# niessner/Opt

Measured on AMD Instinct MI355X. Metric: PCG iters/s, GN solve of image_warping 4096^2, higher is better.
Workload: dtype f32; 1 GPU; image_warping 4096x4096 float, gaussNewtonGPU, 400 PCG iterations per GN step (synthetic cat512-style constraints, border pinned); parallelism=single GPU, step=one Opt_ProblemStep (1 GN iteration)

## Files before the change

opt_amd/csrc/energy_image_warping.hip:

```cpp
#include "energy.h"
#include "iw_device.h"
#include "iw_step.h"
#include "iw_iter.h"
#include "pcg_ring.h"
#include "iw_onchip.h"
#include <cstdint>

namespace optamd {
namespace {

template <class T>
struct ImageWarpingOps : EnergyOps<T> {
    IWArgs<T> A{};
    int cus = 256;
    bool useLattice = true;
    int forceRows = 0, maxWorkgroups = 1 << 30, maxExchangePeriod = 1 << 20;
    ImageWarpingOps(const unsigned* dims) {
        A.W = (int)dims[0]; A.H = (int)dims[1];
        this->usePreconditioner = true;
        this->addUnknown(0, (long)A.W * A.H, 2); this->addUnknown(1, (long)A.W * A.H, 1);
        HIP_CHECK(hipMalloc((void**)&A.flags, (size_t)A.W * A.H));
        HIP_CHECK(hipMalloc((void**)&A.cs, (size_t)A.W * A.H * 2 * sizeof(T)));
        int dev = 0; HIP_CHECK(hipGetDevice(&dev));
        HIP_CHECK(hipDeviceGetAttribute(&cus, hipDeviceAttributeMultiprocessorCount, dev));
        if (const char* e = getenv("OPT_AMD_LATTICE")) useLattice = atoi(e) != 0;
        if (const char* e = getenv("OPT_AMD_SLAB_PERIOD")) maxExchangePeriod = std::max(1, atoi(e));
        if (const char* e = getenv("OPT_AMD_ITER_ROWS")) forceRows = std::max(0, atoi(e));
        if (const char* e = getenv("OPT_AMD_ITER_MAXWG")) maxWorkgroups = std::max(1, atoi(e));
        if (const char* e = getenv("OPT_AMD_ONCHIP_FLAT")) ocFlatMax = std::max(0, atoi(e));
        HIP_CHECK(hipMalloc((void**)&dNotLattice, sizeof(int)));
        HIP_CHECK(hipHostMalloc((void**)&hNotLattice, 64)); *hNotLattice = 0;
        HIP_CHECK(hipEventCreateWithFlags(&bindEvent, hipEventDisableTiming));
    }
    ~ImageWarpingOps() override {
        (void)hipHostFree(hNotLattice); (void)hipEventDestroy(bindEvent);
        (void)hipFree(A.flags); (void)hipFree(A.cs); (void)hipFree(dNotLattice);
// ... 172 lines not shown
        const int gx = divUp(A.W, kStrip);
        int gy, rowsPerGroup;
        splitRows(A.yEnd - A.yBegin, gx, cus * occReset, gy, rowsPerGroup);
        FuseArgs<T> F{};
        F.resetB = b; F.resetPre = pre; F.resetR = r; F.resetZ = z; F.resetBNum = bNum.partials; F.resetQ = q.partials;
        ScopedKernel k(ctx, "PCGStep1+PCGStep2_2ndHalf");
        iw_applyJTJ<T, true, false, true><<<gx * gy, kBlock, 0, ctx.stream>>>(A, delta, nullptr, CtC, nullptr, rowsPerGroup, gx, gy, F);
        bNum.n = gx * gy; q.n = gx * gy;
        return true;
    }
    bool applyJTJFused(const T* pOld, const T* z, T* pNew, T* out, const T* CtC, Reduction* dot, const Reduction& bNum, const double* aNumOld,
                       double* aNumNext, LaunchCtx& ctx) override {
        FuseArgs<T> F{z, pNew, bNum.partials, bNum.n, aNumOld, aNumNext};
        launchApply(pOld, out, CtC, dot, ctx, &F);
        return true;
    }

    static const void* iterKernel(bool lat, bool lmLoop, bool flip, int mode) {
#define IWK(LAT, PRE, LMV, MODE) (flip ? (const void*)iw_pcgIter2<T, LAT, PRE, true, LMV, MODE> : (const void*)iw_pcgIter2<T, LAT, PRE, false, LMV, MODE>)
        if (lmLoop) return lat ? (mode == 1 ? IWK(true, 3, true, 1) : mode == 2 ? IWK(true, 3, true, 2) : IWK(true, 3, true, 0)) : IWK(false, 1, true, 0);
        if (lat) return mode == 1 ? IWK(true, 3, false, 1) : mode == 2 ? IWK(true, 3, false, 2) : IWK(true, 3, false, 0);
        return mode == 1 ? IWK(false, 2, false, 1) : mode == 2 ? IWK(false, 2, false, 2) : IWK(false, 2, false, 0);
#undef IWK
    }
    static int iterBlock(bool lat, bool lmLoop) { return sizeof(T) == 8 ? 256 : lat ? 768 : lmLoop ? 512 : 768; }
    int occIter[4] = {0, 0, 0, 0};
    PcgRing<T> ring; double* lmQState = nullptr;
    struct IterLoop {
        bool gn = false, lmRing = false;
        int sinceExchange = 0;
        int lmPrN = 0;
    } loop;
    bool iterAccepts(bool lmLoop) const { return fits32() && (!this->slab.active || (this->slab.ghost >= 2 && !lmLoop)); }
    IterTraits iterTraits(bool lmLoop) const override {
        IterTraits t;
        const bool ok = iterAccepts(lmLoop);
        t.stateExchange = ok;
        t.takesMail = ok && !lmLoop;
        t.postsItself = ok && !lmLoop && this->slab.active;
        t.slabAvailable = ok;
        return t;
    }
    void beginLoop(LaunchCtx& ctx) {
        resolveLattice();
        if (initPending) { if (initHint && !lattice) launchJtf(false, ctx); initHint = lattice; initPending = false; }
    }
    bool pcgIteration(const PcgIterArgs<T>& a, LaunchCtx& ctx) override {
        const bool lmLoop = a.CtC != nullptr;
        if (!a.pre || !iterAccepts(lmLoop)) return false;
        if (a.first) { beginLoop(ctx); loop = IterLoop{}; }
        PcgIterResult<T>& res = *a.result;
        int ext = 0;
        if (this->slab.active) {
            const int period = std::max(1, std::min(this->slab.ghost - 1, maxExchangePeriod)), j = loop.sinceExchange + 1;
            const bool due = j >= period;
            ext = due ? 0 : this->slab.ghost - j;
            loop.sinceExchange = due ? 0 : j;
            res.exchangeDue = due;
        }
        IWArgs<T> Ax = A;
        Ax.yBegin = std::max(0, A.yBegin - ext); Ax.yEnd = std::min(A.H, A.yEnd + ext);
        const int blk = iterBlock(lattice, lmLoop), L = (lmLoop ? 2 : 0) + (lattice ? 1 : 0);
        if (occIter[L] == 0) {
            HIP_CHECK(hipOccupancyMaxActiveBlocksPerMultiprocessor(&occIter[L], iterKernel(lattice, lmLoop, false, 0), blk, 0));
            occIter[L] = std::max(1, std::min(occIter[L], 8));
        }
        const int gx = divUp(A.W, (blk / kWave) * kSpan2);
        int gy, rowsPerGroup;
        splitRows(Ax.yEnd - Ax.yBegin, gx, cus * occIter[L], gy, rowsPerGroup);
        const bool gn = !lmLoop, lmRing = lmLoop && lattice;
        loop.gn = gn; loop.lmRing = lmRing;
        typename PcgRing<T>::Launch R{};
        if (gn || lmRing) {
            ring.allocate((size_t)A.W * A.H * 3, ctx.stream);
            R = ring.next(a.first != 0, a.afterReset != 0, a.rOld, a.pOld);
        } else { R.flip = ring.nextSweep(a.first != 0); R.pOld = a.pOld; R.rOld = a.rOld; R.pNew = a.pNew; }
        if (gn) {
            res.exchange[0] = R.pNew; res.nExchange = 1;
            if (R.k >= 1) { res.exchange[1] = const_cast<T*>(R.pOld); res.nExchange = 2; }
        }
        if (lmRing) {
            res.p = R.pNew; res.wroteDelta = R.deltaMode == 1;
            if (R.owedP) { res.owedP = R.owedP; res.owedAlpha = R.alphaOut; }
            if (!lmQState) {
                HIP_CHECK(hipMalloc((void**)&lmQState, sizeof(double) * (1 + 2 * (size_t)kMaxPartials)));
                HIP_CHECK(hipMemsetAsync(lmQState, 0, sizeof(double) * (1 + 2 * (size_t)kMaxPartials), ctx.stream));
            }
        }
        IterK<T> K{};
        K.rOld = R.rOld; K.pOld = R.pOld; K.rNew = a.rNew; K.pNew = R.pNew; K.delta = a.delta; K.deltaOut = a.deltaOut ? a.deltaOut : a.delta;
        K.pre = a.pre; K.first = a.first; K.deltaMode = R.deltaMode; K.alphaIn = R.alphaIn; K.alphaOut = R.alphaOut; K.rfree = R.rfree;
        K.CtC = a.CtC; K.b = a.b; K.q = a.q ? a.q->partials : nullptr; K.qTag = a.qTag; K.afterReset = a.afterReset;
        K.betaNum = a.betaNum.partials; K.nBetaNum = a.betaNum.n; K.betaDen = a.betaDen.partials; K.nBetaDen = a.betaDen.n;
        if (lmRing) {
            K.qState = lmQState; K.qInit = a.qInit;
            K.pr = lmQState + 1 + (size_t)(R.k & 1) * kMaxPartials; K.prPrev = lmQState + 1 + (size_t)((R.k & 1) ^ 1) * kMaxPartials; K.nPr = loop.lmPrN;
        }
        K.lmRadius = a.lmRadius; K.lmMin = a.lmMinDiag; K.lmMax = a.lmMaxDiag;
        K.aNumPrev = a.aNumPrev.partials; K.aDenPrev = a.aDenPrev.partials; K.s2Prev = a.s2Prev.partials; K.s3Prev = a.s3Prev.partials;
        K.nNum = a.aNumPrev.n; K.nDen = a.aDenPrev.n; K.n2 = a.s2Prev.n; K.n3 = a.s3Prev.n;
        K.aNum = a.aNum->partials; K.aDen = a.aDen->partials; K.s2 = a.s2->partials; K.s3 = a.s3->partials;
        K.ownBegin = A.yBegin; K.ownEnd = A.yEnd;
        K.mail = MailRefDev{a.mail.words, a.mail.world, a.mail.stride, a.mail.tag, a.mail.timeoutTicks, a.mail.errFlag};
        for (int t = 0; t < 16; ++t) K.post.dst[t] = a.post.dst[t];
        K.post.world = a.post.world; K.post.tag = a.post.tag; K.post.ticket = a.post.ticket;
        K.deltaZero = 0;
        if (deltaZero && !a.first && R.deltaMode != 2 && gn) { K.deltaZero = 1; deltaZero = false; }
        {
            ScopedKernel k(ctx, "PCGIteration");
            int rpg = rowsPerGroup, gxa = gx, gya = gy;
            void* kargs[] = {(void*)&Ax, (void*)&K, (void*)&rpg, (void*)&gxa, (void*)&gya};
            const int mode = ((gn || lmRing) && R.rfree == 1 && !a.first && !a.afterReset && !K.deltaZero) ? (R.deltaMode == 2 ? 1 : 2) : 0;
            HIP_CHECK(hipLaunchKernel(iterKernel(lattice, lmLoop, R.flip != 0, mode), dim3(gx * gy), dim3(blk), kargs, 0, ctx.stream));
        }
        a.aNum->n = a.aDen->n = a.s2->n = a.s3->n = gx * gy;
        if (a.q) a.q->n = lmRing ? 1 : gx * gy;
        loop.lmPrN = gx * gy;
        return true;
    }
    void addOwedTerm(T* delta, const T* p, const T* alpha, LaunchCtx& ctx) override {
        ScopedKernel k(ctx, "PCGStep2_delta");
        const long n = 3L * A.W * A.H;
        axpyDeferred<T><<<flatGrid(n), kBlock, 0, ctx.stream>>>(delta, p, alpha, n);
    }
    const T* pcgFinish(T* delta, LaunchCtx& ctx) override {
        if (deltaZero) { HIP_CHECK(hipMemsetAsync(delta, 0, ((size_t)A.W * A.H * 3 + 3) / 4 * 4 * sizeof(T), ctx.stream)); deltaZero = false; }
        if (!loop.gn) return nullptr;
        const long n = 3L * A.W * A.H;
        return ring.finish(delta, n, flatGrid(n), ctx);
    }
    bool finishUpdate(const T* delta, const Reduction& aNum, const Reduction& aDen, LaunchCtx& ctx) override {
        if (this->slab.active || !loop.gn) return false;
        ScopedKernel k(ctx, "PCGLinearUpdate");
        const long N = (long)A.W * A.H;
        iw_finishUpdate<T><<<flatGrid(N), kBlock, 0, ctx.stream>>>(const_cast<T*>(A.Offset), const_cast<T*>(A.Angle), deltaZero ? nullptr : delta, ring.pLast(), ring.termOwed() ? ring.pPrev() : nullptr,
                                                                   ring.alphaSlot(ring.iterIndex - 1), N, aNum.partials, aNum.n, aDen.partials, aDen.n);
        ring.settled(); deltaZero = false;
        return true;
    }
    bool supportsSlab() const override { return true; }
    long rowScalars(int img) const override { return (long)A.W * (img == 0 ? 2 : 1); }

    struct OcVariant { int rows; bool apLds, deltaGlb; const void* fn; size_t lds; int occ; };
    std::vector<OcVariant> ocVariants, ocVariantsLM, ocVariantsGeneral, ocVariantsGeneralLM;
    OnchipGuard guard;
    OnchipGuard* onChipGuard() override { return &guard; }
    int ocFlatMax = 256; long long* ocProf = nullptr;
    OnchipSync ocS{};
    void ocInit() {
        if (!ocVariants.empty()) return;
// ... 122 lines not shown
    void onChipApply(const T* delta, const double* verdict, bool , LaunchCtx& ctx) override {
        ScopedKernel k(ctx, "PCGLinearUpdate");
        const long N = (long)A.W * A.H;
        iw_applyDelta<T><<<flatGrid(N), kBlock, 0, ctx.stream>>>(const_cast<T*>(A.Offset), const_cast<T*>(A.Angle), delta, N, guard.bad, verdict, guard.hostErr, guard.stepWord());
        guard.launched = true;
    }
    std::string describe(int L, bool lmv, const OnChipLm<T>*) override {
        const Slab& sl = this->slab;
        const int rowsOwned = (sl.active ? sl.yEnd - sl.yBegin : A.H);
        char buf[1400];
        if (sl.active) { A.yBegin = sl.yBegin; A.yEnd = sl.yEnd; } else { A.yBegin = 0; A.yEnd = A.H; }
        int tX = 0, tY = 0;
        const bool eligible = guard.usable() && L > 0 && !(lmv && sl.active);
        const OcVariant* V = eligible ? ocSelect(tX, tY, lmv) : nullptr;
        int uX = 0, uY = 0; const OcVariant* U = nullptr;
        if (eligible && !V && maxWorkgroups < (1 << 30)) { const int keep = maxWorkgroups; maxWorkgroups = 1 << 30; U = ocSelect(uX, uY, lmv); maxWorkgroups = keep; }
        const bool ghostOk = !sl.active || sl.ghost >= 2;
        const long rowBytes = (long)A.W * 3 * (long)sizeof(T);
        const std::string cap = maxWorkgroups < (1 << 30) ? std::to_string(maxWorkgroups) + " (OPT_AMD_ITER_MAXWG: ranks share a GPU)" : std::string("none");
        if (V && ghostOk)
            snprintf(buf, sizeof buf, "path=on-chip (if UrShape is the unit lattice%s); onchip_rows_per_lane=%d; tiles=%dx%d of %d CUs; lds_bytes=%zu; slab_rows=%d; ghost_rows=%d; workgroup_cap=%s; "
                     "per_iteration_cross_rank=%s; fallback=one launch per PCG iteration (iw_pcgIter2)",
                     sl.active ? " and every rank and the communicator agree" : "", V->rows, tX, tY, cus, V->lds, rowsOwned, sl.active ? sl.ghost : 0, cap.c_str(),
                     sl.active ? "edge rows of A p as tagged words (2 x W x 3 scalars x 8 B per neighbour) + one rank hop of 4 doubles, inside the persistent launch" : "none");
        else {
            const std::string why = guard.whyOff() ? guard.whyOff() : (lmv && sl.active) ? "the LM variants are single-GPU" : !ghostOk ? "needs >= 2 ghost rows" :
                                    U ? "the workgroup cap -- without it: on-chip, " + std::to_string(U->rows) + " rows per lane, " + std::to_string(uX) + "x" + std::to_string(uY) + " tiles" :
                                    "the tiles do not fit one per CU (or the slab is no whole number of tiles)";
            const std::string cross = sl.active ? "one all-reduce of 4 doubles, and every " + std::to_string(std::max(1, sl.ghost - 1)) + " iterations " + std::to_string(2L * sl.ghost * rowBytes) +
                                                  " B of edge rows (the two newest search directions) per neighbour" : std::string("none");
            snprintf(buf, sizeof buf, "path=one launch per PCG iteration (iw_pcgIter2%s); why_not_on_chip=%s; slab_rows=%d; ghost_rows=%d; workgroup_cap=%s; per_iteration_cross_rank=%s",
                     lmv ? ", LM" : "", why.c_str(), rowsOwned, sl.active ? sl.ghost : 0, cap.c_str(), cross.c_str());
        }
        if (this->onChipLevel < 4) return buf;
        std::string d = buf;
        int gX = 0, gY = 0;
        const OcVariant* GV = (eligible && !sl.active) ? ocSelect(gX, gY, lmv, true) : nullptr;
        if (GV && lmv && gX * gY > ocFlatMax) GV = nullptr;
        if (GV) {
            if (V && ghostOk) d.replace(0, d.find(';'), "path=on-chip (unit-lattice UrShape: iw_onchipPcg, any other UrShape: iw_onchipPcgGeneral)");
            d += "; general_urshape=on-chip (iw_onchipPcgGeneral" + std::string(lmv ? ", LM" : "") + "), " + std::to_string(GV->rows) + " rows per lane, " + std::to_string(gX) + "x" + std::to_string(gY) +
                 " tiles, " + std::to_string(GV->lds) + " B of LDS";
        } else {
            const std::string why = guard.whyOff() ? guard.whyOff() : sl.active ? "row slabs take the on-chip solve on a unit lattice only" : L <= 0 ? "no PCG iterations" :
                                    "no general-UrShape variant fits one tile per CU (at most " + std::to_string(sizeof(T) == 4 ? 2048 : 1024) + " pixels per CU" + (lmv ? ", LM: at most " + std::to_string(ocFlatMax) + " tiles" : "") + ")";
            d += "; general_urshape=one launch per PCG iteration (iw_pcgIter2" + std::string(lmv ? ", LM" : "") + "); why_not_on_chip_general=" + why;
        }
        return d;
    }
    bool supportsDeferredSteps() const override { return !this->slab.active; }
    bool deltaMovable() const override { return !this->slab.active; }
};

template <class T> EnergyOps<T>* makeIW(const unsigned* dims) { return new ImageWarpingOps<T>(dims); }

}

EnergyInfo imageWarpingInfo() {
    EnergyInfo e;
    e.name = "image_warping"; e.nDims = 2; e.usePreconditioner = true; e.floatOnly = false; e.residualsPerElement = 10;
    e.params = {{ParamDecl::kUnknown, "Offset", "opt_float2", 0}, {ParamDecl::kUnknown, "Angle", "opt_float", 1},
                {ParamDecl::kArray, "UrShape", "opt_float2", 2},  {ParamDecl::kArray, "Constraints", "opt_float2", 3},
                {ParamDecl::kArray, "Mask", "opt_float", 4},      {ParamDecl::kScalar, "w_fitSqrt", "float", 5},
                {ParamDecl::kScalar, "w_regSqrt", "float", 6}};
    e.makeFloat = makeIW<float>; e.makeDouble = makeIW<double>;
    return e;
}

// ... 2 lines not shown
```

opt_amd/csrc/iw_device.h:

```cpp
#pragma once
#include "common.h"
#include <cstdint>

namespace optamd {
namespace {

template <class T> struct V2 { T x, y; };

constexpr uint8_t kActive = 1, kFit = 2;
constexpr int kCountShift = 2;

template <class T>
struct Q {
    T ox, oy, a;
    T c, s;
    T ux, uy;
    T on;
    T fw;
};
template <int DX, int DY, bool LATTICE, class T>
__device__ __forceinline__ void iw_pairQ(const Q<T>& c, const Q<T>& n, T& ax, T& ay, T& aa) {
    T Dcx, Dcy, Dnx, Dny;
    if (LATTICE) {
        Dcx = DX ? T(DX) * c.s : T(DY) * c.c;   Dcy = DX ? T(-DX) * c.c : T(DY) * c.s;
// ... 30 lines not shown
    const T jnx = -dx - Dnx * n.a, jny = -dy - Dny * n.a;
    PairOut<T> o;
    o.dx = jcx - jnx; o.dy = jcy - jny;
    o.tn = Dnx * jnx + Dny * jny;
    ax += n.on * o.dx; ay += n.on * o.dy;
    aa -= n.on * (Dcx * jcx + Dcy * jcy);
    return o;
}
template <class T>
__device__ __forceinline__ void iw_pairInherited(const PairOut<T>& o, T nOn, T& ax, T& ay, T& aa) {
    ax -= nOn * o.dx; ay -= nOn * o.dy;
    aa -= nOn * o.tn;
}
template <class T>
struct IWArgs {
    int W, H;
    int yBegin, yEnd;
    int gy0, Hg;
    const T* Offset; const T* Angle; const T* UrShape; const T* Constraints; const T* Mask;
    T w_fit, w_reg;
    uint8_t* flags;
    T* cs;
};


__device__ __forceinline__ float regCopy(float v) { float r; asm("v_mov_b32 %0, %1" : "=v"(r) : "v"(v)); return r; }
__device__ __forceinline__ int regCopy(int v) { int r; asm("v_mov_b32 %0, %1" : "=v"(r) : "v"(v)); return r; }
__device__ __forceinline__ double regCopy(double v) { return __hiloint2double(regCopy(__double2hiint(v)), regCopy(__double2loint(v))); }


typedef unsigned int iw_u2 __attribute__((ext_vector_type(2)));
typedef unsigned int iw_u4 __attribute__((ext_vector_type(4)));
__device__ __forceinline__ __amdgpu_buffer_rsrc_t iw_rsrc(const void* base) { return __builtin_amdgcn_make_buffer_rsrc(const_cast<void*>(base), 0, -1 , 0x00020000); }
__device__ __forceinline__ V2<float> bufLd2(__amdgpu_buffer_rsrc_t r, unsigned v, unsigned so, const float*) { const iw_u2 w = __builtin_amdgcn_raw_buffer_load_b64(r, (int)v, (int)so, 0); return V2<float>{__uint_as_float(w.x), __uint_as_float(w.y)}; }
__device__ __forceinline__ V2<double> bufLd2(__amdgpu_buffer_rsrc_t r, unsigned v, unsigned so, const double*) { const iw_u4 w = __builtin_amdgcn_raw_buffer_load_b128(r, (int)v, (int)so, 0); V2<double> o; __builtin_memcpy(&o, &w, 16); return o; }
__device__ __forceinline__ float bufLd1(__amdgpu_buffer_rsrc_t r, unsigned v, unsigned so, const float*) { return __uint_as_float(__builtin_amdgcn_raw_buffer_load_b32(r, (int)v, (int)so, 0)); }
__device__ __forceinline__ double bufLd1(__amdgpu_buffer_rsrc_t r, unsigned v, unsigned so, const double*) { const iw_u2 w = __builtin_amdgcn_raw_buffer_load_b64(r, (int)v, (int)so, 0); double o; __builtin_memcpy(&o, &w, 8); return o; }
__device__ __forceinline__ void bufSt2(__amdgpu_buffer_rsrc_t r, unsigned v, unsigned so, float x, float y) { __builtin_amdgcn_raw_buffer_store_b64(iw_u2{__float_as_uint(x), __float_as_uint(y)}, r, (int)v, (int)so, 0); }
__device__ __forceinline__ void bufSt2(__amdgpu_buffer_rsrc_t r, unsigned v, unsigned so, double x, double y) { const V2<double> o{x, y}; iw_u4 w; __builtin_memcpy(&w, &o, 16); __builtin_amdgcn_raw_buffer_store_b128(w, r, (int)v, (int)so, 0); }
__device__ __forceinline__ void bufSt1(__amdgpu_buffer_rsrc_t r, unsigned v, unsigned so, float x) { __builtin_amdgcn_raw_buffer_store_b32(__float_as_uint(x), r, (int)v, (int)so, 0); }
__device__ __forceinline__ void bufSt1(__amdgpu_buffer_rsrc_t r, unsigned v, unsigned so, double x) { iw_u2 w; __builtin_memcpy(&w, &x, 8); __builtin_amdgcn_raw_buffer_store_b64(w, r, (int)v, (int)so, 0); }
}
}
```

opt_amd/csrc/iw_iter.h:

```cpp
#pragma once
#include "iw_device.h"

namespace optamd {
namespace {

constexpr int kSpan2 = kWave - 4;
template <class T, bool LATTICE, int PRE, bool LM> struct IterBlk {
    static constexpr int value = sizeof(T) == 8 ? 256 : LATTICE ? 768 : (PRE == 2 && !LM) ? 768 : 512;
};

template <class T>
struct IterRaw {
    V2<T> ro, po, mo, u, co; T ra, pa, ma, ca, ang;
    int f, ok;
};
template <class T>
struct IterK {
    const T *rOld, *pOld; T *rNew, *pNew; T* delta; T* deltaOut;
    const T* pre;
    int first;
    int deltaMode; const T* alphaIn; T* alphaOut;
    int rfree;
    const T* CtC; const T* b; double* q; unsigned qTag; int afterReset; const double* betaNum; int nBetaNum; const double* betaDen; int nBetaDen;
    double* qState; double qInit;
    const double* prPrev; int nPr; double* pr;
    T lmRadius, lmMin, lmMax;
    const double *aNumPrev, *aDenPrev, *s2Prev, *s3Prev; int nNum, nDen, n2, n3;
    double *aNum, *aDen, *s2, *s3;
    int ownBegin, ownEnd;
    MailRefDev mail;
    MailPostDev post;
    int deltaZero;
};
template <class T>
struct IterBufs {
    __amdgpu_buffer_rsrc_t rOld, pOld, pNew, rNew, delta, deltaOut, angle, flags, pre, ctc, b, ur;
    unsigned x2, x1, x0;
    unsigned aPart;
};
template <class T, bool LATTICE, int PRE, bool LMV, bool FLIP>
__device__ __forceinline__ IterRaw<T> iw_iterLoad(const IWArgs<T>& A, const IterBufs<T>& B, bool xok, int y) {
    IterRaw<T> r;
    r.ok = xok && y >= 0 && y < A.H;
    const int yc = min(max(y, 0), A.H - 1);
    const unsigned row = (unsigned)(FLIP ? A.H - 1 - yc : yc) * (unsigned)A.W;
    const unsigned s2 = row * (unsigned)sizeof(V2<T>), s1 = row * (unsigned)sizeof(T), s1a = s1 + B.aPart;
    const T* tag = nullptr;
    r.f = __builtin_amdgcn_raw_buffer_load_b8(B.flags, (int)B.x0, (int)row, 0);
    r.ro = bufLd2(B.rOld, B.x2, s2, tag); r.ra = bufLd1(B.rOld, B.x1, s1a, tag);
    r.po = bufLd2(B.pOld, B.x2, s2, tag); r.pa = bufLd1(B.pOld, B.x1, s1a, tag);
    if (PRE == 1) { r.mo = bufLd2(B.pre, B.x2, s2, tag); r.ma = bufLd1(B.pre, B.x1, s1a, tag); }
    else { r.mo = V2<T>{0, 0}; r.ma = 0; }
    if (LMV) { r.co = bufLd2(B.ctc, B.x2, s2, tag); r.ca = bufLd1(B.ctc, B.x1, s1a, tag); } else { r.co = V2<T>{0, 0}; r.ca = 0; }
    r.ang = bufLd1(B.angle, B.x1, s1, tag);
    if (LATTICE) r.u = V2<T>{0, 0}; else r.u = bufLd2(B.ur, B.x2, s2, tag);
    return r;
}

template <bool RIGHT, bool LATTICE, class T> __device__ __forceinline__ void dppShiftConst(const Q<T>& p, Q<T>& q) {
    q.c = dppShift<RIGHT>(p.c); q.s = dppShift<RIGHT>(p.s); q.on = dppShift<RIGHT>(p.on);
    if (LATTICE) { q.ux = 0; q.uy = 0; } else { q.ux = dppShift<RIGHT>(p.ux); q.uy = dppShift<RIGHT>(p.uy); }
    q.fw = 0;
}
template <bool RIGHT, class T> __device__ __forceinline__ void dppShiftVec(const Q<T>& p, Q<T>& q) {
    q.ox = dppShift<RIGHT>(p.ox); q.oy = dppShift<RIGHT>(p.oy); q.a = dppShift<RIGHT>(p.a);
}
template <class T>
struct OldRow {
    Q<T> q;
    T rx, ry, ra, mx, my, ma;
    T cx, cy, ca;
    T p2x, p2y, p2a;
};
template <class T>
struct NewRow {
    Q<T> q;
    T rx, ry, ra, mx, my, ma;
    T cx, cy, ca;
    Q<T> lf, rt;
};

template <class T, bool LATTICE, int PRE, bool FLIP, bool LM = false, int MODE = 0>
__global__ __launch_bounds__((IterBlk<T, LATTICE, PRE, LM>::value), 1) void iw_pcgIter2(IWArgs<T> A, IterK<T> K, int rowsPerGroup, int gx, int gy) {
    static_assert(MODE == 0 || !LM || PRE == 3, "steady-state specialisations: the r-free loops (Gauss-Newton; Levenberg-Marquardt on a unit lattice)");
    static_assert(PRE >= 1 && PRE <= 3, "image_warping always preconditions (image_warping.t:10)");
    const int kDeltaMode = MODE == 1 ? 2 : MODE == 2 ? 1 : K.deltaMode, kRfree = MODE ? 1 : K.rfree;
    constexpr bool LMRF = LM && PRE == 3;
    constexpr int kBlk = IterBlk<T, LATTICE, PRE, LM>::value, kStripW = (kBlk / kWave) * kSpan2;
    __shared__ double scratch[5 * (kBlk / kWave + 1)];
    const long N = (long)A.W * A.H;
    const int bx = blockIdx.x % gx, by = blockIdx.x / gx;
    const int lane = threadIdx.x & (kWave - 1), wave = threadIdx.x >> 6;
    const int x = bx * kStripW + wave * kSpan2 + lane - 2;
    const bool xok = x >= 0 && x < A.W;
    const bool writer = xok && lane >= 2 && lane < 2 + kSpan2;
    const int lyBegin = FLIP ? A.H - A.yEnd : A.yBegin, lyEnd = FLIP ? A.H - A.yBegin : A.yEnd;
    const int yb = lyBegin + by * rowsPerGroup, ye = min(yb + rowsPerGroup, lyEnd);
    IterBufs<T> Bf;
    {
        const unsigned xc = (unsigned)min(max(x, 0), A.W - 1);
        Bf.x2 = xc * (unsigned)sizeof(V2<T>); Bf.x1 = xc * (unsigned)sizeof(T); Bf.x0 = xc; Bf.aPart = (unsigned)(2 * N * (long)sizeof(T));
        Bf.rOld = iw_rsrc(K.rOld); Bf.pOld = iw_rsrc(K.pOld); Bf.pNew = iw_rsrc(K.pNew); Bf.rNew = iw_rsrc(K.rNew); Bf.delta = iw_rsrc(K.delta); Bf.deltaOut = iw_rsrc(K.deltaOut);
        Bf.angle = iw_rsrc(A.Angle); Bf.flags = iw_rsrc(A.flags); Bf.pre = iw_rsrc(K.pre); Bf.ctc = iw_rsrc(K.CtC); Bf.b = iw_rsrc(K.b); Bf.ur = iw_rsrc(A.UrShape);
    }
    auto loadRow = [&](int y) { return iw_iterLoad<T, LATTICE, PRE, LM && PRE != 3, FLIP>(A, Bf, xok, y); };
    const IterRaw<T> raw0 = loadRow(yb - 2), raw1 = loadRow(yb - 1);
    IterRaw<T> rwA = loadRow(yb), rwB = loadRow(yb + 1), rwC = loadRow(yb + 2);
    T alpha = 0, beta = 0;
    const bool first = MODE ? false : K.first != 0;
    const bool restart = LM && MODE == 0 && K.afterReset != 0;
    if (restart) {
        const double* const ps[2] = {K.betaNum, K.betaDen}; const int ns[2] = {K.nBetaNum, K.nBetaDen}; double o2[2];
        sumPartialsN<2>(ps, ns, scratch, o2);
        const T bNum = (T)o2[0], bDen = (T)o2[1];
        beta = (bDen > T(0)) ? bNum / bDen : T(0);
    } else if (!first) {
        const double* const ps[4] = {K.aNumPrev, K.aDenPrev, K.s2Prev, K.s3Prev}; const int ns[4] = {K.nNum, K.nDen, K.n2, K.n3}; double o4[4]; double prD = 0;
        if (!LM && K.mail.words) {
            __shared__ double mailScr[4 + 1 + 64];
            pollMailSums<4>(K.mail, mailScr, o4);
        } else if constexpr (LMRF) {
            const double* const ps5[5] = {K.aNumPrev, K.aDenPrev, K.s2Prev, K.s3Prev, K.prPrev}; const int ns5[5] = {K.nNum, K.nDen, K.n2, K.n3, K.nPr}; double o5[5];
            sumPartialsN<5>(ps5, ns5, scratch, o5);
            o4[0] = o5[0]; o4[1] = o5[1]; o4[2] = o5[2]; o4[3] = o5[3]; prD = o5[4];
        } else sumPartialsN<4>(ps, ns, scratch, o4);
        const double aNumD = o4[0], aDenD = o4[1], s2 = o4[2], s3 = o4[3];
        const T aNum = (T)aNumD, aDen = (T)aDenD;
        alpha = (aDen > T(0)) ? aNum / aDen : T(0);
        if (LMRF && blockIdx.x == 0 && threadIdx.x == 0) {
            const double qNow = K.qState[0] + (double)alpha * (prD - 0.5 * (double)alpha * aDenD);
            K.qState[0] = qNow;
            if (K.qTag) storeTaggedPartial(K.q, 0, qNow, K.qTag); else K.q[0] = qNow;
        }
        const double bNumD = fmax(aNumD - 2.0 * (double)alpha * s2 + (double)alpha * (double)alpha * s3, 0.0);
        beta = (aNum > T(0)) ? (T)bNumD / aNum : T(0);
    }
    if (K.alphaOut && blockIdx.x == 0 && threadIdx.x == 0) { K.alphaOut[0] = alpha; K.alphaOut[2] = beta; }
    if (LMRF && (first || restart) && blockIdx.x == 0 && threadIdx.x == 0) K.qState[0] = first ? 0.0 : K.qInit;
    const T alpha2 = (kDeltaMode == 1) ? K.alphaIn[0] : T(0);
    const bool reconR = (!LM || LMRF) && kRfree == 1;
// ... 41 lines not shown
            if (reconR) { ix = iy = iTab[io]; ia = iTab[10 + cnt]; }
        } else if (PRE == 2) {
            o.mx = o.my = mTab[io]; o.ma = 0;
            if (!LM && reconR) { ix = iy = iTab[io]; ia = T(1); }
        } else {
            o.mx = w.mo.x; o.my = w.mo.y; o.ma = w.ma;
            if (!LM && reconR) { ix = T(1) / o.mx; iy = T(1) / o.my; ia = T(1) / o.ma; }
        }
        if ((!LM || LMRF) && LATTICE && kRfree) { o.p2x = w.ro.x; o.p2y = w.ro.y; o.p2a = w.ra; }
        if (reconR) {
            o.rx = (o.q.ox - betaOlder * w.ro.x) * ix; o.ry = (o.q.oy - betaOlder * w.ro.y) * iy; o.ra = (o.q.a - betaOlder * w.ra) * ia;
        }
    };
    auto applyA = [&](const Q<T>& c, const Q<T>& lf, const Q<T>& rt, const Q<T>& prev, const Q<T>& next, PairOut<T>& vert, T& ox, T& oy, T& oa, bool wantM, T& vertM, T& pa) {
        T ax = 0, ay = 0, aa = 0;
        T mh[2] = {0, 0}, mv[2] = {0, 0};
        const PairOut<T> hr = iw_pairFull<1, 0, LATTICE>(c, rt, ax, ay, aa, wantM ? mh : nullptr, A.w_reg);
        PairOut<T> hl; hl.dx = dppShift<true>(hr.dx); hl.dy = dppShift<true>(hr.dy); hl.tn = dppShift<true>(hr.tn);
        const T mhl = wantM ? dppShift<true>(mh[1]) : T(0);
        iw_pairInherited(hl, lf.on, ax, ay, aa);
        if (!FLIP) {
            const PairOut<T> vn = iw_pairFull<0, 1, LATTICE>(c, next, ax, ay, aa, wantM ? mv : nullptr, A.w_reg); iw_pairInherited(vert, prev.on, ax, ay, aa); vert = vn;
            if (wantM) { T t = rt.on * mh[0]; t += lf.on * mhl; t += next.on * mv[0]; t += prev.on * vertM; pa = t; vertM = mv[1]; }
        } else {
            iw_pairInherited(vert, prev.on, ax, ay, aa); vert = iw_pairFull<0, -1, LATTICE>(c, next, ax, ay, aa, wantM ? mv : nullptr, A.w_reg);
            if (wantM) { T t = rt.on * mh[0]; t += lf.on * mhl; t += prev.on * vertM; t += next.on * mv[0]; pa = t; vertM = mv[1]; }
        }
        ox = c.on * (w2 * ax + c.fw * c.ox); oy = c.on * (w2 * ay + c.fw * c.oy); oa = c.on * (w2 * aa);
    };
    PairOut<T> vOld{0, 0, 0}, vNew{0, 0, 0};
    T vOldM = 0, unusedM = 0;
    constexpr bool kDeltaEarly = MODE == 2 || (LM && !LMRF);
    struct DeltaPre { V2<T> o; T a; };
    auto loadDelta = [&](int y1) {
        DeltaPre d{V2<T>{0, 0}, 0};
        if constexpr (kDeltaEarly) {
            const int yc = min(max(y1, 0), A.H - 1);
            const unsigned rowE = (unsigned)(FLIP ? A.H - 1 - yc : yc) * (unsigned)A.W;
            const T* const tag = nullptr;
            d.o = bufLd2(Bf.delta, Bf.x2, rowE * (unsigned)sizeof(V2<T>), tag); d.a = bufLd1(Bf.delta, Bf.x1, rowE * (unsigned)sizeof(T) + Bf.aPart, tag);
            __builtin_amdgcn_sched_barrier(0);
        }
        return d;
    };
    auto trip = [&](int y, const OldRow<T>& oA, const OldRow<T>& oB, const OldRow<T>& oC,
                    const NewRow<T>& nA, const NewRow<T>& nB, NewRow<T>& nC, bool live, const DeltaPre& dPre) {
        nC.q = oB.q;
        nC.lf = Q<T>{}; nC.lf.on = dppShift<true>(oB.q.on);
        dppShiftConst<false, LATTICE>(oB.q, nC.rt);
        Q<T> lf = nC.lf, rt = nC.rt;
        dppShiftVec<false>(oB.q, rt);
        T ax, ay, aa, paB = 0;
        applyA(oB.q, lf, rt, oA.q, oC.q, vOld, ax, ay, aa, PRE == 2, vOldM, paB);
        if (LM) { ax += oB.cx * oB.q.ox; ay += oB.cy * oB.q.oy; aa += oB.ca * oB.q.a; }
        T maB = oB.ma, raB = oB.ra;
        if (PRE == 2) {
            const T sq = T(1) + sqrt(paB), ia = sq * sq;
            maB = T(1) / ia;
            if (!LM && reconR) raB = oB.ra * ia;
        }
        const T rx = keepR ? oB.rx : oB.rx - alpha * ax, ry = keepR ? oB.ry : oB.ry - alpha * ay, ra = keepR ? raB : raB - alpha * aa;
        nC.mx = oB.mx; nC.my = oB.my; nC.ma = maB;
        nC.cx = oB.cx; nC.cy = oB.cy; nC.ca = oB.ca;
        nC.rx = rx; nC.ry = ry; nC.ra = ra;
        const T zx = nC.mx * rx, zy = nC.my * ry, za = nC.ma * ra;
        nC.q.ox = zx + beta * oB.q.ox; nC.q.oy = zy + beta * oB.q.oy; nC.q.a = za + beta * oB.q.a;
        if (live && writer && y + 1 >= yb && y + 1 < ye) {
            const int yp = phys(y + 1);
            const unsigned rowE = (unsigned)yp * (unsigned)A.W, s2 = rowE * (unsigned)sizeof(V2<T>), s1a = rowE * (unsigned)sizeof(T) + Bf.aPart;
            const T* const tag = nullptr;
            const bool own = yp >= K.ownBegin && yp < K.ownEnd;
            if (own && !keepR && kDeltaMode != 2) {
                V2<T> d; T da;
// ... 9 lines not shown
                    }
                }
                d.x += alpha * oB.q.ox; d.y += alpha * oB.q.oy; da += alpha * oB.q.a;
                bufSt2(Bf.deltaOut, Bf.x2, s2, d.x, d.y); bufSt1(Bf.deltaOut, Bf.x1, s1a, da);
                if (LM && !LMRF) {
                    const V2<T> bo = bufLd2(Bf.b, Bf.x2, s2, tag); const T ba = bufLd1(Bf.b, Bf.x1, s1a, tag);
                    accQ += (double)(T(0.5) * (d.x * (rx + bo.x))) + (double)(T(0.5) * (d.y * (ry + bo.y))) + (double)(T(0.5) * (da * (ra + ba)));
                }
            }
            if (!kRfree) { bufSt2(Bf.rNew, Bf.x2, s2, rx, ry); bufSt1(Bf.rNew, Bf.x1, s1a, ra); }
            bufSt2(Bf.pNew, Bf.x2, s2, nC.q.ox, nC.q.oy); bufSt1(Bf.pNew, Bf.x1, s1a, nC.q.a);
        }
        Q<T> l2 = nB.lf, r2 = nB.rt;
        dppShiftVec<false>(nB.q, r2);
        T ox, oy, oa;
        applyA(nB.q, l2, r2, nA.q, nC.q, vNew, ox, oy, oa, false, unusedM, unusedM);
        if (LM) { ox += nB.cx * nB.q.ox; oy += nB.cy * nB.q.oy; oa += nB.ca * nB.q.a; }
        if (live && writer && y >= yb && phys(y) >= K.ownBegin && phys(y) < K.ownEnd) {
            accDen += (double)(nB.q.ox * ox + nB.q.oy * oy + nB.q.a * oa);
            if (LMRF) accQ += (double)nB.q.ox * (double)nB.rx + (double)nB.q.oy * (double)nB.ry + (double)nB.q.a * (double)nB.ra;
            const double mx = (double)nB.mx, my = (double)nB.my, ma = (double)nB.ma;
            const double rx2 = (double)nB.rx, ry2 = (double)nB.ry, ra2 = (double)nB.ra, ax2 = (double)ox, ay2 = (double)oy, az2 = (double)oa;
            const double mrx = mx * rx2, mry = my * ry2, mra = ma * ra2;
            accNum += mrx * rx2 + mry * ry2 + mra * ra2;
            acc2 += mrx * ax2 + mry * ay2 + mra * az2;
            acc3 += (mx * ax2) * ax2 + (my * ay2) * ay2 + (ma * az2) * az2;
        }
    };
    OldRow<T> o0, o1, o2;
    NewRow<T> n0{}, n1{}, n2{};
    makeOld(raw0, o0);
    makeOld(raw1, o1);
    { T t0 = 0, t1 = 0, t2 = 0, m0[2] = {0, 0}; vOld = iw_pairFull<0, FLIP ? -1 : 1, LATTICE>(o0.q, o1.q, t0, t1, t2, PRE == 2 ? m0 : nullptr, A.w_reg); vOldM = m0[1]; }
    DeltaPre dlA = loadDelta(yb - 1), dlB = dlA, dlC = dlA;
    for (int y = yb - 2; y < ye; y += 3) {
        __syncthreads();
        { makeOld(rwA, o2); dlB = loadDelta(y + 2); rwA = loadRow(y + 5); trip(y, o0, o1, o2, n0, n1, n2, true, dlA); }
        { makeOld(rwB, o0); dlC = loadDelta(y + 3); rwB = loadRow(y + 6); trip(y + 1, o1, o2, o0, n1, n2, n0, y + 1 < ye, dlB); }
        { makeOld(rwC, o1); dlA = loadDelta(y + 4); rwC = loadRow(y + 7); trip(y + 2, o2, o0, o1, n2, n0, n1, y + 2 < ye, dlC); }
    }
    double v[5] = {accDen, accNum, acc2, acc3, accQ};
    blockReduceSumN<5>(v, scratch);
    if (threadIdx.x == 0) {
        K.aDen[blockIdx.x] = v[0]; K.aNum[blockIdx.x] = v[1]; K.s2[blockIdx.x] = v[2]; K.s3[blockIdx.x] = v[3];
        if (LMRF) K.pr[blockIdx.x] = v[4];
        else if (LM) { if (K.qTag) storeTaggedPartial(K.q, blockIdx.x, v[4], K.qTag); else K.q[blockIdx.x] = v[4]; }
    }
    if (!LM && K.post.world) {
        double* const parts[4] = {K.aNum, K.aDen, K.s2, K.s3};
        postMailSums<4>(K.post, parts, scratch);
    }
}

}
}
```

Measured before the change: 5859 PCG iters/s.

## Tile PCG iteration per wave column with balanced row groups and records-masked loads

Replaces the 2D grid of workgroup strips with a flat assignment of waves to (column, row-group) units. Row groups are balanced so the long groups get one extra row, and the loop runs a uniform trip count. Dead waves and past-end trips are masked by building buffer resources with zero records instead of branching, so their loads return zero without touching memory. The aim is to cut tail imbalance and wasted fetches on partial workgroups, at the cost of rebuilding buffer descriptors per load and adding some integer arithmetic.

```diff
diff --git a/opt_amd/csrc/energy_image_warping.hip b/opt_amd/csrc/energy_image_warping.hip
--- a/opt_amd/csrc/energy_image_warping.hip
+++ b/opt_amd/csrc/energy_image_warping.hip
@@ -2,6 +2,7 @@
 #include "iw_device.h"
 #include "iw_step.h"
 #include "iw_iter.h"
+#include "iw_tiling.h"
 #include "pcg_ring.h"
 #include "iw_onchip.h"
 #include <cstdint>
@@ -240,6 +241,14 @@
         int lmPrN = 0;
     } loop;
     bool iterAccepts(bool lmLoop) const { return fits32() && (!this->slab.active || (this->slab.ghost >= 2 && !lmLoop)); }
+    IterTiling iterTilingFor(int rows, bool lat, bool lmLoop) {
+        const int blk = iterBlock(lat, lmLoop), L = (lmLoop ? 2 : 0) + (lat ? 1 : 0);
+        if (occIter[L] == 0) {
+            HIP_CHECK(hipOccupancyMaxActiveBlocksPerMultiprocessor(&occIter[L], iterKernel(lat, lmLoop, false, 0), blk, 0));
+            occIter[L] = std::max(1, std::min(occIter[L], 8));
+        }
+        return iterTiling(A.W, rows, blk / kWave, cus * occIter[L] * (blk / kWave), std::min(maxWorkgroups, kMaxPartials), forceRows);
+    }
     IterTraits iterTraits(bool lmLoop) const override {
         IterTraits t;
         const bool ok = iterAccepts(lmLoop);
@@ -268,14 +277,7 @@
         }
         IWArgs<T> Ax = A;
         Ax.yBegin = std::max(0, A.yBegin - ext); Ax.yEnd = std::min(A.H, A.yEnd + ext);
-        const int blk = iterBlock(lattice, lmLoop), L = (lmLoop ? 2 : 0) + (lattice ? 1 : 0);
-        if (occIter[L] == 0) {
-            HIP_CHECK(hipOccupancyMaxActiveBlocksPerMultiprocessor(&occIter[L], iterKernel(lattice, lmLoop, false, 0), blk, 0));
-            occIter[L] = std::max(1, std::min(occIter[L], 8));
-        }
-        const int gx = divUp(A.W, (blk / kWave) * kSpan2);
-        int gy, rowsPerGroup;
-        splitRows(Ax.yEnd - Ax.yBegin, gx, cus * occIter[L], gy, rowsPerGroup);
+        const IterTiling tile = iterTilingFor(Ax.yEnd - Ax.yBegin, lattice, lmLoop);
         const bool gn = !lmLoop, lmRing = lmLoop && lattice;
         loop.gn = gn; loop.lmRing = lmRing;
         typename PcgRing<T>::Launch R{};
@@ -316,14 +318,14 @@
         if (deltaZero && !a.first && R.deltaMode != 2 && gn) { K.deltaZero = 1; deltaZero = false; }
         {
             ScopedKernel k(ctx, "PCGIteration");
-            int rpg = rowsPerGroup, gxa = gx, gya = gy;
-            void* kargs[] = {(void*)&Ax, (void*)&K, (void*)&rpg, (void*)&gxa, (void*)&gya};
+            int rpg = tile.rowsPerGroup, longGroups = tile.longGroups, cols = tile.cols, units = tile.units, trips = tile.trips;
+            void* kargs[] = {(void*)&Ax, (void*)&K, (void*)&rpg, (void*)&longGroups, (void*)&cols, (void*)&units, (void*)&trips};
             const int mode = ((gn || lmRing) && R.rfree == 1 && !a.first && !a.afterReset && !K.deltaZero) ? (R.deltaMode == 2 ? 1 : 2) : 0;
-            HIP_CHECK(hipLaunchKernel(iterKernel(lattice, lmLoop, R.flip != 0, mode), dim3(gx * gy), dim3(blk), kargs, 0, ctx.stream));
-        }
-        a.aNum->n = a.aDen->n = a.s2->n = a.s3->n = gx * gy;
-        if (a.q) a.q->n = lmRing ? 1 : gx * gy;
-        loop.lmPrN = gx * gy;
+            HIP_CHECK(hipLaunchKernel(iterKernel(lattice, lmLoop, R.flip != 0, mode), dim3(tile.workgroups), dim3(iterBlock(lattice, lmLoop)), kargs, 0, ctx.stream));
+        }
+        a.aNum->n = a.aDen->n = a.s2->n = a.s3->n = tile.workgroups;
+        if (a.q) a.q->n = lmRing ? 1 : tile.workgroups;
+        loop.lmPrN = tile.workgroups;
         return true;
     }
     void addOwedTerm(T* delta, const T* p, const T* alpha, LaunchCtx& ctx) override {
@@ -512,8 +514,14 @@
             snprintf(buf, sizeof buf, "path=one launch per PCG iteration (iw_pcgIter2%s); why_not_on_chip=%s; slab_rows=%d; ghost_rows=%d; workgroup_cap=%s; per_iteration_cross_rank=%s",
                      lmv ? ", LM" : "", why.c_str(), rowsOwned, sl.active ? sl.ghost : 0, cap.c_str(), cross.c_str());
         }
-        if (this->onChipLevel < 4) return buf;
         std::string d = buf;
+        if (fits32()) {
+            const IterTiling t = iterTilingFor(rowsOwned, useLattice, lmv);
+            d += "; iteration_tiling=" + std::to_string(t.cols) + " wave columns x " + std::to_string(t.groups) + " row groups, " + std::to_string(t.rowsPerGroup) + " rows per group (" + std::to_string(t.longGroups) + " groups, the others one less), " +
+                 std::to_string(t.trips) + " trips, " + std::to_string(t.workgroups) + " workgroups of " + std::to_string(iterBlock(useLattice, lmv) / kWave) + " waves" +
+                 (useLattice ? " (unit-lattice UrShape)" : "");
+        }
+        if (this->onChipLevel < 4) return d;
         int gX = 0, gY = 0;
         const OcVariant* GV = (eligible && !sl.active) ? ocSelect(gX, gY, lmv, true) : nullptr;
         if (GV && lmv && gX * gY > ocFlatMax) GV = nullptr;
diff --git a/opt_amd/csrc/iw_device.h b/opt_amd/csrc/iw_device.h
--- a/opt_amd/csrc/iw_device.h
+++ b/opt_amd/csrc/iw_device.h
@@ -86,6 +86,8 @@
 typedef unsigned int iw_u2 __attribute__((ext_vector_type(2)));
 typedef unsigned int iw_u4 __attribute__((ext_vector_type(4)));
 __device__ __forceinline__ __amdgpu_buffer_rsrc_t iw_rsrc(const void* base) { return __builtin_amdgcn_make_buffer_rsrc(const_cast<void*>(base), 0, -1 , 0x00020000); }
+__device__ __forceinline__ int iw_records(bool fetch) { return __builtin_amdgcn_readfirstlane(fetch ? -1 : 0); }
+__device__ __forceinline__ __amdgpu_buffer_rsrc_t iw_rsrc(const void* base, int records) { return __builtin_amdgcn_make_buffer_rsrc(const_cast<void*>(base), 0, records, 0x00020000); }
 __device__ __forceinline__ V2<float> bufLd2(__amdgpu_buffer_rsrc_t r, unsigned v, unsigned so, const float*) { const iw_u2 w = __builtin_amdgcn_raw_buffer_load_b64(r, (int)v, (int)so, 0); return V2<float>{__uint_as_float(w.x), __uint_as_float(w.y)}; }
 __device__ __forceinline__ V2<double> bufLd2(__amdgpu_buffer_rsrc_t r, unsigned v, unsigned so, const double*) { const iw_u4 w = __builtin_amdgcn_raw_buffer_load_b128(r, (int)v, (int)so, 0); V2<double> o; __builtin_memcpy(&o, &w, 16); return o; }
 __device__ __forceinline__ float bufLd1(__amdgpu_buffer_rsrc_t r, unsigned v, unsigned so, const float*) { return __uint_as_float(__builtin_amdgcn_raw_buffer_load_b32(r, (int)v, (int)so, 0)); }
diff --git a/opt_amd/csrc/iw_iter.h b/opt_amd/csrc/iw_iter.h
--- a/opt_amd/csrc/iw_iter.h
+++ b/opt_amd/csrc/iw_iter.h
@@ -1,10 +1,12 @@
 #pragma once
 #include "iw_device.h"
+#include "iw_tiling.h"
 
 namespace optamd {
 namespace {
 
 constexpr int kSpan2 = kWave - 4;
+static_assert(kSpan2 == kIterSpan, "iw_tiling.h cuts the image into columns of the width a wave produces");
 template <class T, bool LATTICE, int PRE, bool LM> struct IterBlk {
     static constexpr int value = sizeof(T) == 8 ? 256 : LATTICE ? 768 : (PRE == 2 && !LM) ? 768 : 512;
 };
@@ -34,26 +36,28 @@
 };
 template <class T>
 struct IterBufs {
-    __amdgpu_buffer_rsrc_t rOld, pOld, pNew, rNew, delta, deltaOut, angle, flags, pre, ctc, b, ur;
+    __amdgpu_buffer_rsrc_t rOld, pNew, rNew, delta, deltaOut, b;
+    const void *rOldP, *pOldP, *deltaP, *angleP, *flagsP, *preP, *ctcP, *urP;
     unsigned x2, x1, x0;
     unsigned aPart;
 };
 template <class T, bool LATTICE, int PRE, bool LMV, bool FLIP>
-__device__ __forceinline__ IterRaw<T> iw_iterLoad(const IWArgs<T>& A, const IterBufs<T>& B, bool xok, int y) {
+__device__ __forceinline__ IterRaw<T> iw_iterLoad(const IWArgs<T>& A, const IterBufs<T>& B, bool xok, int y, int records) {
     IterRaw<T> r;
     r.ok = xok && y >= 0 && y < A.H;
     const int yc = min(max(y, 0), A.H - 1);
     const unsigned row = (unsigned)(FLIP ? A.H - 1 - yc : yc) * (unsigned)A.W;
     const unsigned s2 = row * (unsigned)sizeof(V2<T>), s1 = row * (unsigned)sizeof(T), s1a = s1 + B.aPart;
     const T* tag = nullptr;
-    r.f = __builtin_amdgcn_raw_buffer_load_b8(B.flags, (int)B.x0, (int)row, 0);
-    r.ro = bufLd2(B.rOld, B.x2, s2, tag); r.ra = bufLd1(B.rOld, B.x1, s1a, tag);
-    r.po = bufLd2(B.pOld, B.x2, s2, tag); r.pa = bufLd1(B.pOld, B.x1, s1a, tag);
-    if (PRE == 1) { r.mo = bufLd2(B.pre, B.x2, s2, tag); r.ma = bufLd1(B.pre, B.x1, s1a, tag); }
+    const __amdgpu_buffer_rsrc_t rOld = iw_rsrc(B.rOldP, records), pOld = iw_rsrc(B.pOldP, records);
+    r.f = __builtin_amdgcn_raw_buffer_load_b8(iw_rsrc(B.flagsP, records), (int)B.x0, (int)row, 0);
+    r.ro = bufLd2(rOld, B.x2, s2, tag); r.ra = bufLd1(rOld, B.x1, s1a, tag);
+    r.po = bufLd2(pOld, B.x2, s2, tag); r.pa = bufLd1(pOld, B.x1, s1a, tag);
+    if (PRE == 1) { const __amdgpu_buffer_rsrc_t pre = iw_rsrc(B.preP, records); r.mo = bufLd2(pre, B.x2, s2, tag); r.ma = bufLd1(pre, B.x1, s1a, tag); }
     else { r.mo = V2<T>{0, 0}; r.ma = 0; }
-    if (LMV) { r.co = bufLd2(B.ctc, B.x2, s2, tag); r.ca = bufLd1(B.ctc, B.x1, s1a, tag); } else { r.co = V2<T>{0, 0}; r.ca = 0; }
-    r.ang = bufLd1(B.angle, B.x1, s1, tag);
-    if (LATTICE) r.u = V2<T>{0, 0}; else r.u = bufLd2(B.ur, B.x2, s2, tag);
+    if (LMV) { const __amdgpu_buffer_rsrc_t ctc = iw_rsrc(B.ctcP, records); r.co = bufLd2(ctc, B.x2, s2, tag); r.ca = bufLd1(ctc, B.x1, s1a, tag); } else { r.co = V2<T>{0, 0}; r.ca = 0; }
+    r.ang = bufLd1(iw_rsrc(B.angleP, records), B.x1, s1, tag);
+    if (LATTICE) r.u = V2<T>{0, 0}; else r.u = bufLd2(iw_rsrc(B.urP, records), B.x2, s2, tag);
     return r;
 }
 
@@ -81,31 +85,35 @@
 };
 
 template <class T, bool LATTICE, int PRE, bool FLIP, bool LM = false, int MODE = 0>
-__global__ __launch_bounds__((IterBlk<T, LATTICE, PRE, LM>::value), 1) void iw_pcgIter2(IWArgs<T> A, IterK<T> K, int rowsPerGroup, int gx, int gy) {
+__global__ __launch_bounds__((IterBlk<T, LATTICE, PRE, LM>::value), 1) void iw_pcgIter2(IWArgs<T> A, IterK<T> K, int rowsPerGroup, int longGroups, int cols, int units, int trips) {
     static_assert(MODE == 0 || !LM || PRE == 3, "steady-state specialisations: the r-free loops (Gauss-Newton; Levenberg-Marquardt on a unit lattice)");
     static_assert(PRE >= 1 && PRE <= 3, "image_warping always preconditions (image_warping.t:10)");
     const int kDeltaMode = MODE == 1 ? 2 : MODE == 2 ? 1 : K.deltaMode, kRfree = MODE ? 1 : K.rfree;
     constexpr bool LMRF = LM && PRE == 3;
-    constexpr int kBlk = IterBlk<T, LATTICE, PRE, LM>::value, kStripW = (kBlk / kWave) * kSpan2;
+    constexpr int kBlk = IterBlk<T, LATTICE, PRE, LM>::value;
     __shared__ double scratch[5 * (kBlk / kWave + 1)];
     const long N = (long)A.W * A.H;
-    const int bx = blockIdx.x % gx, by = blockIdx.x / gx;
-    const int lane = threadIdx.x & (kWave - 1), wave = threadIdx.x >> 6;
-    const int x = bx * kStripW + wave * kSpan2 + lane - 2;
-    const bool xok = x >= 0 && x < A.W;
+    const int lane = threadIdx.x & (kWave - 1), wave = __builtin_amdgcn_readfirstlane((int)(threadIdx.x >> 6));
+    const IterUnit unit = iterUnit((int)blockIdx.x, kBlk / kWave, wave, cols, units);
+    const int x = unit.col * kSpan2 + lane - 2;
+    const bool xok = unit.live && x >= 0 && x < A.W;
     const bool writer = xok && lane >= 2 && lane < 2 + kSpan2;
     const int lyBegin = FLIP ? A.H - A.yEnd : A.yBegin, lyEnd = FLIP ? A.H - A.yBegin : A.yEnd;
-    const int yb = lyBegin + by * rowsPerGroup, ye = min(yb + rowsPerGroup, lyEnd);
+    const int nRows = lyEnd - lyBegin;
+    const int yb = lyBegin + (unit.live ? iterGroupBegin(unit.group, rowsPerGroup, longGroups) : nRows);
+    const int ye = lyBegin + (unit.live ? iterGroupEnd(unit.group, rowsPerGroup, longGroups, nRows) : nRows);
     IterBufs<T> Bf;
     {
         const unsigned xc = (unsigned)min(max(x, 0), A.W - 1);
         Bf.x2 = xc * (unsigned)sizeof(V2<T>); Bf.x1 = xc * (unsigned)sizeof(T); Bf.x0 = xc; Bf.aPart = (unsigned)(2 * N * (long)sizeof(T));
-        Bf.rOld = iw_rsrc(K.rOld); Bf.pOld = iw_rsrc(K.pOld); Bf.pNew = iw_rsrc(K.pNew); Bf.rNew = iw_rsrc(K.rNew); Bf.delta = iw_rsrc(K.delta); Bf.deltaOut = iw_rsrc(K.deltaOut);
-        Bf.angle = iw_rsrc(A.Angle); Bf.flags = iw_rsrc(A.flags); Bf.pre = iw_rsrc(K.pre); Bf.ctc = iw_rsrc(K.CtC); Bf.b = iw_rsrc(K.b); Bf.ur = iw_rsrc(A.UrShape);
-    }
-    auto loadRow = [&](int y) { return iw_iterLoad<T, LATTICE, PRE, LM && PRE != 3, FLIP>(A, Bf, xok, y); };
-    const IterRaw<T> raw0 = loadRow(yb - 2), raw1 = loadRow(yb - 1);
-    IterRaw<T> rwA = loadRow(yb), rwB = loadRow(yb + 1), rwC = loadRow(yb + 2);
+        Bf.rOld = iw_rsrc(K.rOld); Bf.pNew = iw_rsrc(K.pNew); Bf.rNew = iw_rsrc(K.rNew); Bf.delta = iw_rsrc(K.delta); Bf.deltaOut = iw_rsrc(K.deltaOut);
+        Bf.b = iw_rsrc(K.b);
+        Bf.rOldP = K.rOld; Bf.pOldP = K.pOld; Bf.deltaP = K.delta; Bf.angleP = A.Angle; Bf.flagsP = A.flags; Bf.preP = K.pre; Bf.ctcP = K.CtC; Bf.urP = A.UrShape;
+    }
+    const int nDelta = unit.live ? ye - yb : 0, nFetch = unit.live ? ye - yb + 4 : 0;
+    auto loadRow = [&](int k) { return iw_iterLoad<T, LATTICE, PRE, LM && PRE != 3, FLIP>(A, Bf, xok, yb - 2 + k, iw_records(k < nFetch)); };
+    const IterRaw<T> raw0 = loadRow(0), raw1 = loadRow(1);
+    IterRaw<T> rwA = loadRow(2), rwB = loadRow(3), rwC = loadRow(4);
     T alpha = 0, beta = 0;
     const bool first = MODE ? false : K.first != 0;
     const bool restart = LM && MODE == 0 && K.afterReset != 0;
@@ -213,13 +221,15 @@
     T vOldM = 0, unusedM = 0;
     constexpr bool kDeltaEarly = MODE == 2 || (LM && !LMRF);
     struct DeltaPre { V2<T> o; T a; };
-    auto loadDelta = [&](int y1) {
+    auto loadDelta = [&](int k) {
         DeltaPre d{V2<T>{0, 0}, 0};
         if constexpr (kDeltaEarly) {
+            const int y1 = yb - 2 + k;
             const int yc = min(max(y1, 0), A.H - 1);
             const unsigned rowE = (unsigned)(FLIP ? A.H - 1 - yc : yc) * (unsigned)A.W;
             const T* const tag = nullptr;
-            d.o = bufLd2(Bf.delta, Bf.x2, rowE * (unsigned)sizeof(V2<T>), tag); d.a = bufLd1(Bf.delta, Bf.x1, rowE * (unsigned)sizeof(T) + Bf.aPart, tag);
+            const __amdgpu_buffer_rsrc_t delta = iw_rsrc(Bf.deltaP, iw_records((unsigned)(k - 2) < (unsigned)nDelta));
+            d.o = bufLd2(delta, Bf.x2, rowE * (unsigned)sizeof(V2<T>), tag); d.a = bufLd1(delta, Bf.x1, rowE * (unsigned)sizeof(T) + Bf.aPart, tag);
             __builtin_amdgcn_sched_barrier(0);
         }
         return d;
@@ -295,12 +305,12 @@
     makeOld(raw0, o0);
     makeOld(raw1, o1);
     { T t0 = 0, t1 = 0, t2 = 0, m0[2] = {0, 0}; vOld = iw_pairFull<0, FLIP ? -1 : 1, LATTICE>(o0.q, o1.q, t0, t1, t2, PRE == 2 ? m0 : nullptr, A.w_reg); vOldM = m0[1]; }
-    DeltaPre dlA = loadDelta(yb - 1), dlB = dlA, dlC = dlA;
-    for (int y = yb - 2; y < ye; y += 3) {
+    DeltaPre dlA = loadDelta(1), dlB = dlA, dlC = dlA;
+    for (int t = 0, y = yb - 2; t < trips; t += 3, y += 3) {
         __syncthreads();
-        { makeOld(rwA, o2); dlB = loadDelta(y + 2); rwA = loadRow(y + 5); trip(y, o0, o1, o2, n0, n1, n2, true, dlA); }
-        { makeOld(rwB, o0); dlC = loadDelta(y + 3); rwB = loadRow(y + 6); trip(y + 1, o1, o2, o0, n1, n2, n0, y + 1 < ye, dlB); }
-        { makeOld(rwC, o1); dlA = loadDelta(y + 4); rwC = loadRow(y + 7); trip(y + 2, o2, o0, o1, n2, n0, n1, y + 2 < ye, dlC); }
+        { makeOld(rwA, o2); dlB = loadDelta(t + 2); rwA = loadRow(t + 5); trip(y, o0, o1, o2, n0, n1, n2, y < ye, dlA); }
+        { makeOld(rwB, o0); dlC = loadDelta(t + 3); rwB = loadRow(t + 6); trip(y + 1, o1, o2, o0, n1, n2, n0, y + 1 < ye, dlB); }
+        { makeOld(rwC, o1); dlA = loadDelta(t + 4); rwC = loadRow(t + 7); trip(y + 2, o2, o0, o1, n2, n0, n1, y + 2 < ye, dlC); }
     }
     double v[5] = {accDen, accNum, acc2, acc3, accQ};
     blockReduceSumN<5>(v, scratch);
diff --git a/opt_amd/csrc/iw_tiling.h b/opt_amd/csrc/iw_tiling.h
--- /dev/null
+++ b/opt_amd/csrc/iw_tiling.h
@@ -0,0 +1,54 @@
+#pragma once
+
+namespace optamd {
+
+constexpr int kIterSpan = 60;
+
+struct IterTiling {
+    int cols;
+    int groups;
+    int rowsPerGroup;
+    int longGroups;
+    int units;
+    int workgroups;
+    int trips;
+};
+
+constexpr int iterGroupBegin(int g, int rowsPerGroup, int longGroups) { return g * rowsPerGroup - (g > longGroups ? g - longGroups : 0); }
+constexpr int iterGroupEnd(int g, int rowsPerGroup, int longGroups, int rows) {
+    const int e = iterGroupBegin(g, rowsPerGroup, longGroups) + rowsPerGroup - (g >= longGroups ? 1 : 0);
+    return e < rows ? e : rows;
+}
+
+struct IterUnit { int col, group; bool live; };
+constexpr IterUnit iterUnit(int workgroup, int wavesPerWG, int wave, int cols, int units) {
+    const int u = workgroup * wavesPerWG + wave;
+    return IterUnit{u % cols, u / cols, u < units};
+}
+
+inline IterTiling iterTiling(int W, int rows, int wavesPerWG, int slots, int maxWorkgroups, int forceRows) {
+    const auto divUp = [](long a, long b) { return (a + b - 1) / b; };
+    IterTiling t;
+    t.cols = (int)divUp(W, kIterSpan);
+    const long capUnits = (long)(maxWorkgroups < 1 ? 1 : maxWorkgroups) * wavesPerWG;
+    const long maxGroups = capUnits / t.cols < 1 ? 1 : capUnits / t.cols;
+    long g = (slots < capUnits ? slots : capUnits) / t.cols;
+    g = g < 1 ? 1 : g > rows ? rows : g;
+    long rpg = divUp(rows, g);
+    t.longGroups = (int)(rows - g * (rpg - 1));
+    if (forceRows > 0) {
+        rpg = forceRows < rows ? forceRows : rows;
+        const long floorRows = divUp(rows, maxGroups);
+        if (rpg < floorRows) rpg = floorRows;
+        g = divUp(rows, rpg);
+        t.longGroups = (int)g;
+    }
+    t.rowsPerGroup = (int)rpg;
+    t.groups = (int)g;
+    t.units = t.cols * t.groups;
+    t.workgroups = (int)divUp(t.units, wavesPerWG);
+    t.trips = 3 * (int)divUp(rpg + 2, 3);
+    return t;
+}
+
+}
```

Result: slower. 5754 PCG iters/s (-1.8%).
